# medvedevgroup/TwoPaCo

Measured on AMD Instinct MI355X. Metric: kmers_hashed_per_sec, higher is better.
Workload: dtype u64

## Files before the change

### twopaco_amd/csrc/tpc_capi.hip

```cpp
#include "tpc_ctx.h"

namespace tpch {

int fail(tpc_ctx *c, int code, const char *fmt, ...)
{
    char buf[512];
    va_list ap;
    va_start(ap, fmt);
    vsnprintf(buf, sizeof buf, fmt, ap);
    va_end(ap);
    if (c) c->err = buf;
    return code;
}





TpcLaunch make_launch(const tpc_ctx *c)
{
    TpcLaunch a;
    a.P = c->P; a.tab = c->tab; a.bases = c->bases; a.nmask = c->nmask; a.n_text = c->n_text;
    a.n_tiles = c->n_tiles; a.filter = c->filter; a.stream = c->stream;
    a.stat_kernel = c->stat_kernel;
    return a;
}

TpcLaunch make_launch_periodic(const tpc_ctx *c)
{
    TpcLaunch a = make_launch(c);
    if (c->periodic && c->periodic_valid) {
        if (c->periodic_any_q) a.per_qs = c->periodic;
        if (c->periodic_any_i) a.per_i = c->periodic + (size_t)(1 + TPC_PER_PLANES) * c->n_words_alloc;
    }
    return a;
}

void ensure_periodic(tpc_ctx *c)
{
    if (c->periodic_valid || !c->opt_periodic || !c->bases || !c->have_params || c->n_words_alloc == 0) return;
    if ((c->sh_world > 1 || c->text_windowed) && !c->opt_shard_periodic && !replicated(c)) return;
    TpcLaunch a = make_launch(c);
    const uint64_t w0 = c->text_windowed ? c->text_w0 : 0, w1 = c->text_windowed ? std::min(c->text_w1, c->n_words) : c->n_words;
    const uint64_t pos_hi = c->text_windowed ? c->text_w1 << 5 : ~0ull;
    uint32_t any[2] = {0, 0};
    uint32_t *flags = reinterpret_cast<uint32_t *>(c->counters + 6);
    if (hipMemsetAsync(flags, 0, sizeof any, c->stream) != hipSuccess) return;
    tpc_launch_periodic_build(a, nullptr, nullptr, 0, nullptr, w0, w1, w0 << 5, pos_hi, flags);
    if (hipMemcpyAsync(any, flags, sizeof any, hipMemcpyDeviceToHost, c->stream) != hipSuccess || hipStreamSynchronize(c->stream) != hipSuccess) return;
    c->periodic_any_q = any[0] != 0; c->periodic_any_i = any[1] != 0;
    if (any[0] || any[1]) {
        const size_t words = (size_t)(2 + TPC_PER_PLANES) * c->n_words_alloc;
        if (!c->periodic && hipMalloc((void **)&c->periodic, words * sizeof(uint32_t)) != hipSuccess) { (void)hipGetLastError(); c->periodic = nullptr; return; }
        if (hipMemsetAsync(c->periodic, 0, words * sizeof(uint32_t), c->stream) != hipSuccess) return;
        tpc_launch_periodic_build(a, c->periodic, c->periodic + c->n_words_alloc, c->n_words_alloc, c->periodic + (size_t)(1 + TPC_PER_PLANES) * c->n_words_alloc, w0, w1, w0 << 5, pos_hi, flags);
        if (hipStreamSynchronize(c->stream) != hipSuccess) return;
    }
// ... 194 lines not shown
        n = c->rmask_sums_n;
    } else {
        c->rmask_sums_valid = false;
        tpc_launch_mask_count(c->stream, m, c->n_words, c->block_sums, c->counters + 2);
        if ((rc = read_counter(c, 2, &n))) return rc;
    }
    rc = ensure(c, c->marks, c->marks_cap, n);
    if (rc) return rc;
    if (n) tpc_launch_mask_scatter(c->stream, m, c->n_words, c->block_sums, c->marks);
    c->n_marks = n;
    return 0;
}

}

extern "C" {

int tpc_ctx_create(int device, tpc_ctx **out)
{
    if (!out) return -1;
    *out = nullptr;
    int n = 0;
    if (hipGetDeviceCount(&n) != hipSuccess || n <= 0) return -2;
    if (device < 0 || device >= n) return -3;
    if (hipSetDevice(device) != hipSuccess) return -4;
    tpc_ctx *c = new tpc_ctx();
    c->device = device;
    c->dbg_ovf = getenv("TPC_DEBUG_OVF") != nullptr; c->dbg_phases = getenv("TPC_PROFILE_PHASES") != nullptr; c->dbg_timing = getenv("TWOPACO_TIMING") != nullptr; c->no_lean = TpcEnv::get().no_lean;
    if (const char *e = getenv("TPC_SHARD_TIGHT")) c->opt_shard_tight = atoi(e) ? 1 : 0;
    if (hipStreamCreate(&c->stream) != hipSuccess) { delete c; return -5; }
    for (int i = 0; i < TPC_K_COUNT; i++) {
        if (hipEventCreate(&c->ev0[i]) != hipSuccess || hipEventCreate(&c->ev1[i]) != hipSuccess) { delete c; return -5; }
    }
    if (hipMalloc((void **)&c->tab, TPC_TAB_WORDS * sizeof(uint64_t)) != hipSuccess ||
        hipMalloc((void **)&c->counters, 8 * sizeof(unsigned long long)) != hipSuccess ||
        hipMalloc((void **)&c->route_scratch, 128 * sizeof(unsigned long long)) != hipSuccess) { delete c; return -6; }
    *out = c;
    return 0;
}

void tpc_ctx_destroy(tpc_ctx *c)
{
    if (!c) return;
    (void)hipSetDevice(c->device);
    (void)hipStreamSynchronize(c->stream);
    void *ptrs[] = { c->tab, c->bases_alloc, c->nmask_alloc, c->filter, c->rmask, c->mask, c->marks, c->block_sums, c->table,
                     c->keys, c->idtab, c->emit_id, c->stream_buf, c->counters, c->route_scratch, c->sh_off, c->scan_blocks, c->sort_scratch, c->seg.name, c->seg.first, c->seg.ev[0], c->seg.ev[1], c->seg.ev[2],
                     c->seg.rec, c->seg.amb, c->text_plan.off, c->text_plan.piece, c->text_names, c->text_win };
    for (void *p : ptrs) if (p) (void)hipFree(p);
    stream_part_release(c);
    colors_drop(c);
    links_drop(c);
    anchors_drop(c);
    edges_drop(c);
    for (void *p : c->pbuf) if (p) (void)hipFree(p);
    for (void *p : c->ikeep) if (p) (void)hipFree(p);
    if (c->periodic) (void)hipFree(c->periodic);
    if (c->cmb_base) (void)hipFree(c->cmb_base);
    if (c->cmb_cur) (void)hipFree(c->cmb_cur);
    if (c->ikeep_ovf) (void)hipFree(c->ikeep_ovf);
    if (c->iovf_cnt) (void)hipFree(c->iovf_cnt);
    if (c->iovf_off) (void)hipFree(c->iovf_off);
    for (int i = 0; i < TPC_K_COUNT; i++) { if (c->ev0[i]) (void)hipEventDestroy(c->ev0[i]); if (c->ev1[i]) (void)hipEventDestroy(c->ev1[i]); }
    if (c->stream2) (void)hipStreamDestroy(c->stream2);
    if (c->stream) (void)hipStreamDestroy(c->stream);
    delete c;
}

const char *tpc_last_error(const tpc_ctx *c) { return c ? c->err.c_str() : "null context"; }

int tpc_set_option(tpc_ctx *c, const char *name, int64_t value)
{
    if (!c || !name) return -1;
    if (!strcmp(name, "insert_test_first")) { c->opt_test_first = value != 0; return 0; }
    if (!strcmp(name, "insert_mode")) { c->opt_insert_mode = (int)value; return 0; }
    if (!strcmp(name, "slice_bits")) { c->opt_slice_bits = (int)value; return 0; }
    if (!strcmp(name, "query_mode")) { c->opt_query_mode = (int)value; return 0; }
    if (!strcmp(name, "part_budget_bytes")) { c->opt_part_budget = value; return 0; }
    if (!strcmp(name, "part_levels")) { c->opt_part_levels = (int)value; return 0; }
    if (!strcmp(name, "shard_tight_regions")) { c->opt_shard_tight = value ? 1 : 0; c->sh_have[0] = c->sh_have[1] = false; return 0; }
    if (!strcmp(name, "part_min_tiles")) { c->opt_part_min_tiles = value < 1 ? 1 : value; return 0; }
    if (!strcmp(name, "verify_marks")) { c->opt_verify_marks = value != 0; return 0; }
    if (!strcmp(name, "mark_bucket_bits")) { tpc_test_mark_bucket_bits = (int)value; return 0; }
    if (!strcmp(name, "mark_region_cap")) { tpc_test_mark_region_cap = (int)value; return 0; }
    if (!strcmp(name, "mark_slice_bits")) { tpc_test_mark_slice_bits = (int)value; return 0; }
    if (!strcmp(name, "qhash_pushes")) { tpc_opt_qhash_pushes = value == 8 ? 8 : 6; return 0; }
    if (!strcmp(name, "qhash_roll_scalars")) { tpc_opt_qhash_roll = value != 0; return 0; }
    if (!strcmp(name, "fuse_apply_lookup")) { c->opt_fuse = value != 0; return 0; }
    if (!strcmp(name, "test_q6_pb2")) { tpc_test_q6_pb2 = (int)value; return 0; }
    if (!strcmp(name, "insert_entry_fmt")) { tpc_test_insert_p3 = value == 3; return 0; }
    if (!strcmp(name, "shard_periodic_skip")) { c->opt_shard_periodic = value != 0; return 0; }
    if (!strcmp(name, "periodic_skip")) { c->opt_periodic = value != 0; if (!value) c->periodic_valid = false; return 0; }
    if (!strcmp(name, "test_tight_pinch")) { tpc_test_tight_pinch = (int)value; c->sh_have[0] = c->sh_have[1] = false; return 0; }
    if (!strcmp(name, "test_sched_cap")) { tpc_test_sched_cap = value > 0 ? (uint32_t)value : 0; return 0; }
    if (!strcmp(name, "text_window")) { c->opt_text_window = value != 0; return 0; }
    if (!strcmp(name, "replicate_filter")) { c->opt_replicate = value != 0; return 0; }
    if (!strcmp(name, "test_force_anyq")) { tpc_test_force_anyq = value != 0; return 0; }
    if (!strcmp(name, "test_sketch_grid")) { tpc_test_sketch_grid = value > 0 ? (int)value : 0; return 0; }
    if (!strcmp(name, "test_links_slots_log2")) { c->opt_links_slots_log2 = (int)std::max<int64_t>(-1, std::min<int64_t>(value, 64)); return 0; }
    if (!strcmp(name, "test_edges_slots_log2")) { c->opt_edges_slots_log2 = (int)std::max<int64_t>(-1, std::min<int64_t>(value, 64)); return 0; }
    if (!strcmp(name, "test_edges_hash_bits")) { c->opt_edges_hash_bits = (int)std::max<int64_t>(-1, std::min<int64_t>(value, 65)); return 0; }
    if (!strcmp(name, "test_locate_grid")) { c->opt_locate_grid = value > 0 ? (int)std::min<int64_t>(value, 1 << 20) : 0; return 0; }
    if (!strcmp(name, "test_distances_chunk_words")) { c->opt_distances_chunk_words = (int)std::max<int64_t>(-1, std::min<int64_t>(value, 1 << 20)); return 0; }
    if (!strcmp(name, "test_components_step_limit")) { c->opt_components_step_limit = (int)std::max<int64_t>(-1, std::min<int64_t>(value, 0x7FFFFFFF)); return 0; }
    if (!strcmp(name, "test_fail_mallocs")) { tpc_test_fail_mallocs.store(value > 0 ? (int)value : 0); return 0; }
    return fail(c, -1, "unknown option %s", name);
}

int tpc_preload(int device)
{
    if (hipSetDevice(device) != hipSuccess) { (void)hipGetLastError(); return -10; }
    const bool timing = getenv("TWOPACO_TIMING") != nullptr;
    int (*const warm[4])() = { tpc_warm_partition, tpc_warm_qpartition, tpc_warm_pass2, tpc_warm_stream };
    const char *const name[4] = { "partition", "qpartition", "pass2", "stream" };
    for (int i = 0; i < 4; i++) {
        const auto t0 = std::chrono::steady_clock::now();
        if (warm[i]() != 0) return -10;
        if (timing) fprintf(stderr, "[timing]     code object %s: %.1f ms\n", name[i], std::chrono::duration<double, std::milli>(std::chrono::steady_clock::now() - t0).count());
    }
    return 0;
}

int tpc_warmup(tpc_ctx *c)
{
    if (!c) return -1;
    return tpc_preload(c->device);
}

int64_t tpc_get_stat(const tpc_ctx *c, const char *name)
{
    if (!c || !name) return -1;
    if (!strcmp(name, "insert_path")) return c->stat_path[0];
    if (!strcmp(name, "query_path")) return c->stat_path[1];
    if (!strcmp(name, "insert_entry_fmt")) return c->stat_fmt[0];
    if (!strcmp(name, "query_entry_fmt")) return c->stat_fmt[1];
    if (!strcmp(name, "insert_hash_kernel")) return c->stat_kernel[0];
    if (!strcmp(name, "query_hash_kernel")) return c->stat_kernel[1];
    if (!strcmp(name, "query_verify_kernel")) return c->stat_kernel[2];
    if (!strcmp(name, "query_hash_form")) return c->stat_kernel[3];
    if (!strcmp(name, "query_mark_path")) return c->stat_mark_path;
    if (!strcmp(name, "query_mark_fallback")) return c->stat_mark_fallback;
    if (!strcmp(name, "insert_batches")) return c->stat_batches[0];
    if (!strcmp(name, "query_batches")) return c->stat_batches[1];
    if (!strcmp(name, "query_tiles_per_batch")) return c->stat_q_plan[0];
    if (!strcmp(name, "query_b1")) return c->stat_q_plan[1];
    if (!strcmp(name, "query_b2")) return c->stat_q_plan[2];
    if (!strcmp(name, "query_begun")) return c->stat_q_begun;
    if (!strcmp(name, "filter2_retries")) return c->stat_filter2_retries;
    if (!strcmp(name, "aggregate_retries")) return c->stat_aggregate_retries;
    if (!strcmp(name, "filter2_counted")) return c->stat_filter2_counted;
    if (!strcmp(name, "fused_lookups")) return c->stat_fused;
    if (!strcmp(name, "query_overflow_entries")) return c->stat_query_overflow;
    if (!strcmp(name, "insert_overflow_entries")) return c->stat_insert_overflow;
    if (!strcmp(name, "periodic_skip")) return c->periodic_valid ? 1 : 0;
    if (!strcmp(name, "pbuf_releases")) return c->stat_pbuf_releases;
    if (!strcmp(name, "distances_tile")) return TPC_DISTANCES_TILE;
    if (!strcmp(name, "text_words")) return (int64_t)(c->text_w1 - c->text_w0);
    if (!strcmp(name, "text_word_begin")) return (int64_t)c->text_w0;
    if (!strcmp(name, "text_word_end")) return (int64_t)c->text_w1;
    if (!strcmp(name, "periodic_any_query")) return c->periodic_valid && c->periodic_any_q ? 1 : 0;
    if (!strcmp(name, "periodic_any_insert")) return c->periodic_valid && c->periodic_any_i ? 1 : 0;
    if (!strcmp(name, "text_write_us")) return c->text_write_us;
    if (!strcmp(name, "text_wait_us")) return c->text_wait_us;
    if (!strcmp(name, "text_window_bytes")) return c->text_window_bytes;
    if (!strcmp(name, "device_free_bytes") || !strcmp(name, "device_total_bytes")) {
        size_t free_b = 0, total_b = 0;
        if (hipSetDevice(c->device) != hipSuccess || hipMemGetInfo(&free_b, &total_b) != hipSuccess) { (void)hipGetLastError(); return -1; }
        return (int64_t)(name[7] == 'f' ? free_b : total_b);
    }
    if (!strcmp(name, "round_marks")) return c->marks_valid ? (int64_t)c->n_marks : -1;
    return -1;
}

int tpc_set_params(tpc_ctx *c, int k, int L, int q, const uint64_t *seed_table)
{
    if (!c || !seed_table) return -1;
    if (q < 1 || q > TPC_MAX_Q) return fail(c, -1, "q=%d unsupported (1..%d)", q, TPC_MAX_Q);
    if (L < 2 || L > 62) return fail(c, -1, "filter bits L=%d unsupported (2..62)", L);
    if (k < 1) return fail(c, -1, "k must be positive");
    const int C = (k + 4 + 31) / 32;
    if (C >= 20)
        return fail(c, -1, "The value of K is too big. Please refer to documentaion how to increase the max supported value of K.");
    HIPCHK(c, hipSetDevice(c->device));
    c->P.k = k; c->P.L = L; c->P.q = q; c->P.rk = k % L; c->P.lmask = (1ull << L) - 1ull;
    if (C != c->C && c->keys) {
        (void)hipFree(c->keys);
        c->keys = nullptr; c->keys_cap = 0;
    }
    c->C = C;
    memset(c->tab_host, 0, sizeof c->tab_host);
    for (int i = 0; i < q; i++)
        for (int ch = 0; ch < 5; ch++) {
            const uint64_t h = seed_table[i * 5 + ch];
            if (h > c->P.lmask) return fail(c, -1, "seed table entry exceeds L bits");
            c->tab_host[i * 5 + ch] = h;
            c->tab_host[TPC_TAB_HK + i * 5 + ch] = rotln_host(h, L, c->P.rk);
        }
    HIPCHK(c, hipMemcpy(c->tab, c->tab_host, sizeof c->tab_host, hipMemcpyHostToDevice));
    const uint64_t fw = filter_words_for(L, c->opt_replicate ? 1 : c->sh_world);
    c->sh_have[0] = c->sh_have[1] = false;
    c->pending_lists = false; c->cmb_have_geo = false;
    if (fw != c->filter_words) {
        if (c->filter) (void)hipFree(c->filter);
        c->filter = nullptr;
        HIPCHK(c, hipMalloc((void **)&c->filter, fw * sizeof(uint32_t)));
        c->filter_words = fw;
    }
    c->have_params = true;
    c->periodic_valid = false;
    c->pending_apply = false;
    c->qb_valid = false;
    c->n_keys = 0; c->finalized = false; c->rounds_done = 0; c->mask_dirty = false; c->marks_valid = false; c->rmask_sums_valid = false;
    return 0;
}

int tpc_seq_upload(tpc_ctx *c, const uint64_t *bases, const uint32_t *nmask, uint64_t n_text)
{
    if (!c || !bases || !nmask || n_text < 2) return fail(c, -1, "bad text");
    HIPCHK(c, hipSetDevice(c->device));
    const auto t_begin = std::chrono::steady_clock::now();
    c->qb_valid = false;
    const uint64_t nw = (n_text + 31) / 32;
    if (!((nmask[0] & 1u) && ((nmask[(n_text - 1) >> 5] >> ((n_text - 1) & 31)) & 1u)))
        return fail(c, -1, "text must start and end with the N separator");
    const uint64_t tiles = (nw + TPC_TILE_THREADS - 1) / TPC_TILE_THREADS;
    const uint64_t alloc = ((n_text / TPC_RUN + 512) / 512) * 512 + TPC_XW_MAX + 2;
    uint64_t w0 = 0, w1 = alloc;
    const bool windowed = c->opt_text_window && c->sh_world > 1;
    if (windowed) {
        const uint64_t t512 = (n_text / TPC_RUN + 512) / 512, chunk = (t512 + c->sh_world - 1) / c->sh_world;
// ... 609 lines not shown
```

### twopaco_amd/csrc/tpc_ctx.h

```cpp
#pragma once
#include "../../include/twopaco_hip.h"
#include "tpc_internal.h"

#include <algorithm>
#include <atomic>
#include <cmath>
#include <chrono>
#include <cstdarg>
#include <cstdio>
#include <cstdlib>
#include <cstring>
#include <string>
#include <vector>
#include <map>

struct tpc_ctx {
    __attribute__((always_inline)) tpc_ctx() = default;
    int device = 0;
    hipStream_t stream = nullptr;
    std::string err;
    bool have_params = false;
    TpcHashParams P{};
    uint64_t tab_host[TPC_TAB_WORDS]{};
    uint64_t *tab = nullptr;
    int C = 1;
    uint64_t *bases = nullptr;
    uint32_t *nmask = nullptr;
    uint64_t n_text = 0, n_words = 0, n_words_alloc = 0, n_tiles = 0;
    uint64_t text_uploads = 0;
    uint32_t *periodic = nullptr;
    bool periodic_valid = false;
    bool periodic_any_q = false, periodic_any_i = false;
    int opt_periodic = 1;
    bool opt_shard_periodic = false;
    uint64_t *bases_alloc = nullptr;
    uint32_t *nmask_alloc = nullptr;
    int opt_text_window = 0;
    bool text_windowed = false;
    uint64_t text_w0 = 0, text_w1 = 0;
    uint32_t *filter = nullptr;
    uint64_t filter_words = 0;
    uint32_t *rmask = nullptr, *mask = nullptr;
    bool mask_dirty = false;
    int rounds_done = 0;
    uint64_t *marks = nullptr;
    uint64_t marks_cap = 0, n_marks = 0;
    bool marks_valid = false;
    bool rmask_sums_valid = false;
    uint64_t rmask_sums_n = 0;
    uint64_t *block_sums = nullptr;
    uint64_t *scan_blocks = nullptr;
    void *table = nullptr;
    uint64_t table_cap = 0, table_alloc = 0;
    uint64_t *keys = nullptr;
    uint64_t n_keys = 0, keys_cap = 0;
    bool finalized = false;
// ... 97 lines not shown
        bool valid = false;
    } edg;
    struct Locate {
        unsigned long long *hit = nullptr;
        uint32_t *row = nullptr;
        uint32_t *runs = nullptr;
        unsigned long long *recs = nullptr;
        unsigned long long *shared = nullptr;
        uint64_t positions = 0, windows = 0, found = 0, n_runs = 0, n_rec = 0, peak_bytes = 0;
        uint32_t n_colors = 0;
        bool valid = false;
    } loc;
    int opt_edges_slots_log2 = 0;
    int opt_edges_hash_bits = 0;
    int opt_locate_grid = 0;
    int opt_components_step_limit = 0;
    int opt_distances_chunk_words = 0;
    unsigned long long *counters = nullptr;
    unsigned long long *route_scratch = nullptr;
    uint64_t *sh_off = nullptr;
    size_t sh_off_bytes = 0;
    int opt_test_first = 0;
    int opt_insert_mode = 0;
    int opt_slice_bits = 20;
    bool filter_zero_pending = false;
    static constexpr int NPBUF = 19;
    void *pbuf[NPBUF] = {};
    size_t pbytes[NPBUF] = {};
    std::vector<uint64_t> off2_uploaded, off3_uploaded;
    int opt_part_levels = 0;
    int opt_shard_tight = 1;
    int stat_path[2] = {0, 0};
    int64_t stat_batches[2] = {0, 0};
    mutable int stat_kernel[4] = {0, 0, 0, 0};
    int stat_fmt[2] = {0, 0};
    int64_t stat_filter2_retries = 0;
    int64_t stat_aggregate_retries = 0;
    int stat_filter2_counted = 0;
    int opt_verify_marks = 1;
    int stat_mark_path = 0;
    int64_t stat_mark_fallback = 0;
    int64_t opt_part_min_tiles = 256;
    int64_t opt_part_budget = 0;
    int opt_query_mode = 0;
    int opt_fuse = 1;
    bool pending_apply = false;
    bool pending_fresh = false;
    bool pending_shard = false;
    TpcPartPlan pending_pl;
    void *ikeep[2] = {nullptr, nullptr};
    size_t ikeep_bytes[2] = {0, 0};
    uint64_t *ikeep_ovf = nullptr;
    uint64_t ikeep_ovf_cap = 0;
    uint64_t pending_novf = 0;
    uint32_t *iovf_cnt = nullptr;
    uint64_t *iovf_off = nullptr;
    uint32_t iovf_slices = 0;
    int64_t stat_fused = 0;
    int64_t stat_query_overflow = 0;
    int64_t stat_insert_overflow = 0;
    int64_t stat_pbuf_releases = 0;
    uint32_t sh_rank = 0, sh_world = 1;
    TpcPartPlan sh_ipl;
    TpcQPlan sh_qpl;
    bool sh_have[2] = {false, false};
    uint64_t sh_per[2] = {0, 0}, sh_batches[2] = {0, 0};
    uint64_t sh_nsurv = 0;
// ... 91 lines not shown
```

### twopaco_amd/csrc/tpc_internal.h

```cpp
#pragma once
#include "tpc_device.h"
#include <algorithm>
#include <cstdlib>
#include <vector>

struct TpcEnv {
    bool no_lean, rb_hash, verify_eager, gated_full;
    int verify_marks;
    int qhash_pushes, qhash_roll;
    int ppr_insert, gated_loads, split_loads9;
    int slice_grid;
    static const TpcEnv &get()
    {
        static const TpcEnv e = [] {
            TpcEnv v;
            v.no_lean = getenv("TPC_NO_LEAN") != nullptr;
            v.rb_hash = getenv("TPC_RB_HASH") != nullptr;
            const char *lz = getenv("TPC_VERIFY_LAZY");
            v.verify_eager = lz && lz[0] == '0';
            v.gated_full = getenv("TPC_GATED_FULL_REGIONS") != nullptr;
            const char *vm = getenv("TPC_VERIFY_MARKS");
            v.verify_marks = vm && vm[0] ? (vm[0] != '0' ? 1 : 0) : -1;
            const char *qp = getenv("TPC_QHASH_PUSHES");
            v.qhash_pushes = qp && (atoi(qp) == 6 || atoi(qp) == 8) ? atoi(qp) : 0;
            const char *qr = getenv("TPC_QHASH_ROLL_SCALARS");
            v.qhash_roll = qr && qr[0] ? (qr[0] != '0' ? 1 : 0) : -1;
            const char *p = getenv("TPC_PPR_INSERT"), *g = getenv("TPC_GATED_LOADS");
            v.ppr_insert = p ? atoi(p) : 0;
            v.gated_loads = g ? atoi(g) : 0;
            const char *s9 = getenv("TPC_SPLIT_LOADS9");
            v.split_loads9 = s9 ? atoi(s9) : 0;
            const char *lg = getenv("TPC_LOOKUP_GRID");
            int n_cu = 0, dev = 0;
            if (hipGetDevice(&dev) != hipSuccess || hipDeviceGetAttribute(&n_cu, hipDeviceAttributeMultiprocessorCount, dev) != hipSuccess || n_cu <= 0) { (void)hipGetLastError(); n_cu = 256; }
            v.slice_grid = lg ? atoi(lg) : 2 * n_cu;
            return v;
        }();
        return e;
    }
};

inline uint32_t tpc_slice_grid(uint32_t n_slices)
{
    const int g = TpcEnv::get().slice_grid;
    return g > 0 ? std::min<uint32_t>(n_slices, (uint32_t)g) : n_slices;
}

extern int tpc_opt_qhash_pushes, tpc_opt_qhash_roll;
inline bool tpc_qhash_roll_scalars() { const int e = TpcEnv::get().qhash_roll; return (e >= 0 ? e : tpc_opt_qhash_roll) != 0; }
inline bool tpc_qhash_compact() { const int e = TpcEnv::get().qhash_pushes; return (e ? e : tpc_opt_qhash_pushes) != 8; }

#define TPC_TAB_MAXQ 64
#define TPC_KERNEL_MAXQ 16
#define TPC_TAB_HK (TPC_TAB_MAXQ * 5)
#define TPC_TAB_WORDS (2 * TPC_TAB_MAXQ * 5)

struct TpcLaunch {
    TpcHashParams P;
    const uint64_t *tab;
    const uint64_t *bases;
    const uint32_t *nmask;
    uint64_t n_text;
    uint64_t n_tiles;
    uint32_t *filter;
    hipStream_t stream;
    const uint32_t *per_i = nullptr, *per_qs = nullptr;
    uint64_t g_begin = 0, g_end = ~0ull;
    hipEvent_t ev_lookup0 = nullptr, ev_lookup1 = nullptr;
    int *stat_kernel = nullptr;
};
constexpr int TPC_PER_MAXP = 63;
constexpr int TPC_PER_PLANES = 6;
int tpc_launch_periodic_build(const TpcLaunch &a, uint32_t *qs, uint32_t *qd, uint64_t stride, uint32_t *ins, uint64_t w_begin, uint64_t w_end, uint64_t pos_lo, uint64_t pos_hi,
                              uint32_t *any);
int tpc_launch_periodic_copy(hipStream_t stream, uint32_t *rmask, const uint32_t *qs, const uint32_t *qd, uint64_t stride, uint64_t n_words);

int tpc_launch_insert(const TpcLaunch &a, uint64_t lo, uint64_t hi, bool gated, bool test, unsigned long long *n_kmers);
int tpc_launch_query(const TpcLaunch &a, uint32_t *rmask, uint64_t lo, uint64_t hi, bool gated, unsigned long long *n_marks);
int tpc_launch_split(const TpcLaunch &a, uint32_t *emask, uint32_t *bins, uint64_t bin_size);
int tpc_launch_split_emask(hipStream_t s, const uint64_t *d_rec_start, const uint64_t *d_rec_len, uint32_t n_rec, int k, uint64_t n_words, uint32_t *emask);
int tpc_launch_hash_dump(const TpcLaunch &a, uint64_t g0, uint64_t n, uint64_t *out);
int tpc_launch_insert_anyq(const TpcLaunch &a, uint64_t lo, uint64_t hi, bool gated, bool test, unsigned long long *n_kmers);
int tpc_launch_query_anyq(const TpcLaunch &a, uint32_t *rmask, uint64_t lo, uint64_t hi, bool gated, unsigned long long *n_marks);
int tpc_launch_split_anyq(const TpcLaunch &a, uint32_t *emask, uint32_t *bins, uint64_t bin_size);
extern int tpc_test_force_anyq;

struct TpcPartPlan {
    int slice_bits, b1, b2, pos_per_round;
    int b3 = 0;
    uint32_t perm_mult, perm_inv;
    uint64_t tile0, n_tiles;
    uint32_t nwg1, wpb;
// ... 207 lines not shown
```

### twopaco_amd/csrc/tpc_qpartition.hip

```cpp
#ifndef TPC_QPARTITION_PART
#define TPC_QPARTITION_PART 0
#endif
#include "tpc_rbins.h"
#include "tpc_bins3.h"
#include "tpc_binsp.h"
#include "tpc_lean.h"
#include "tpc_internal.h"
#include "tpc_lists.h"
#include <algorithm>
#include <type_traits>
#include <cstdio>
#include <cstdlib>
#include <cmath>

#if TPC_QPARTITION_PART == 0
int tpc_test_q6_pb2 = 0;
int tpc_opt_qhash_pushes = 6, tpc_opt_qhash_roll = 1;
int tpc_test_mark_bucket_bits = 0, tpc_test_mark_region_cap = 0, tpc_test_mark_slice_bits = 0;
#endif

namespace {

constexpr int QE_E_SHIFT = 31;
constexpr uint64_t QE_REM_MASK = (1ull << QE_E_SHIFT) - 1ull;
constexpr int QS_LISTS = 64;

struct QOverflow {
    uint64_t *list;
    unsigned long long *cursor;
    uint64_t cap;
    __device__ __forceinline__ void push(uint64_t addr, uint64_t sid, int site = 0) const
    {
#ifdef TPC_PROFILE_PHASES
        atomicAdd(cursor + 24 + site, 1ull);
#endif
        const unsigned long long o = atomicAdd(cursor, 1ull);
        if (o < cap) { list[2 * o] = addr; list[2 * o + 1] = sid; } else cursor[1] = 1ull;
    }
};

__device__ __forceinline__ bool within(uint64_t v, uint64_t lo, uint64_t hi) { return v >= lo && v <= hi; }

constexpr int QH_THREADS = 1024;
constexpr int QH_RUN = 16;

__device__ __forceinline__ uint64_t q_rotl_n(uint64_t x, int L, int r)
{
    if (r == 0) return x;
    return ((x & ((1ull << (L - r)) - 1ull)) << r) | (x >> (L - r));
}
// ... 110 lines not shown
#pragma unroll
                            for (int c = 0; c < 4; c++) {
                                {
                                    const uint64_t a0 = perm.fwd(tpc_min(hk0[c] ^ v.pos[0], r1n ^ h0[3 - c]));
                                    eb[c] = (uint32_t)(a0 >> shift);
                                    ev[c] = (a0 & (((uint64_t)1 << shift) - 1)) | ((sid_g | (uint64_t)c) << QE_E_SHIFT);
                                    eok[c] = c != c_prev;
                                }
                                {
                                    const uint64_t a0 = perm.fwd(tpc_min(r1p ^ h0[c], v.neg[0] ^ hk0[3 - c]));
                                    eb[4 + c] = (uint32_t)(a0 >> shift);
                                    ev[4 + c] = (a0 & (((uint64_t)1 << shift) - 1)) | ((sid_g | (uint64_t)(4 + c)) << QE_E_SHIFT);
                                    eok[4 + c] = c != c_next;
                                }
                            }
                            bins.template push_batch<8>(eb, ev, eok, lost);
                        }
                    }
                    v.pos[0] = r1p ^ s_h[c_next] ^ s_hk[c_first];
                    v.neg[0] = tpc_rotr1(v.neg[0] ^ s_hk[tpc_rc(c_next)] ^ s_h[tpc_rc(c_first)], P.L);
                    ncnt += (c_next == TPC_CODE_N) - (c_first == TPC_CODE_N);
                    c_prev = c_first;
                    c_first = c_first_nx;
                }
            }
            bins.template flush<false>(lost);
        }
        rmask16[(wfirst * 2) + tid] = (uint16_t)word;
    }
    if constexpr (RB) { bins.flush(true, reg, lost); bins.store_counts(cnt1, reg, ridx); }
    else { bins.template flush<true>(lost); bins.store_counts(cnt1, ridx); }
}

constexpr int QT_MAXK = 64;
constexpr uint32_t QH_ROLL_S = 1u;

__device__ __forceinline__ uint64_t q_spread2(uint32_t m)
{
    uint64_t x = m;
    x = (x | (x << 16)) & 0x0000FFFF0000FFFFull;
    x = (x | (x << 8)) & 0x00FF00FF00FF00FFull;
    x = (x | (x << 4)) & 0x0F0F0F0F0F0F0F0Full;
    x = (x | (x << 2)) & 0x3333333333333333ull;
    x = (x | (x << 1)) & 0x5555555555555555ull;
    return x | (x << 1);
}

template <bool GATED, bool SHARDED, bool HALF, bool LHI, bool PUSH6>
__global__ void __launch_bounds__(QH_THREADS)
k_q_hash2(int LOG_NB, TpcHashParams P, const uint64_t *__restrict__ tab, const uint64_t *__restrict__ bases,
          const uint32_t *__restrict__ nmask, uint64_t n_text, uint64_t tile0, uint64_t n_tiles, int pos_per_round,
          uint64_t lo, uint64_t hi, uint64_t *buf1, uint32_t *cnt1, uint64_t cap1, QOverflow ovf, PtPerm perm, PtShard sh,
          uint64_t gbase, uint32_t *__restrict__ rmask, uint32_t tiles_per_wg, const uint16_t *__restrict__ skip16, uint32_t mode)
{
    using V = LeanV<LHI>;
    extern __shared__ __attribute__((aligned(16))) unsigned char smem[];
    const int NB = 1 << LOG_NB;
    constexpr int TW = PT_THREADS + 1 + TPC_XW_MAX;
    Bins3<uint64_t, QH_THREADS> bins;
    uint64_t *s_b = reinterpret_cast<uint64_t *>(bins.carve(smem, LOG_NB));
    uint64_t *s_roll = s_b + TW;
    uint64_t *s_seed = s_roll + 20;
    uint32_t *s_n = reinterpret_cast<uint32_t *>(s_seed + QT_MAXK * 10);
    const uint32_t tid = threadIdx.x;
    const int k = P.k, L = P.L;
    if (tid < 5) {
        const uint32_t c = tid, rc = c == 4 ? 4u : 3u - c;
        s_roll[c * 2] = tab[c]; s_roll[c * 2 + 1] = tab[TPC_TAB_HK + rc];
        s_roll[10 + c * 2] = tab[TPC_TAB_HK + c]; s_roll[10 + c * 2 + 1] = tab[rc];
    }
    if (k <= QT_MAXK)
        for (uint32_t i = tid; i < 5u * (uint32_t)k; i += QH_THREADS) {
            const uint32_t t = i / 5u, c = i % 5u, rc = c == 4 ? 4u : 3u - c;
            s_seed[2 * i] = q_rotl_n(tab[c], L, (k - 1 - (int)t) % L);
            s_seed[2 * i + 1] = q_rotl_n(tab[rc], L, (int)t % L);
        }
    const int shift = L - LOG_NB;
    const uint32_t wg = blockIdx.x, nwg = gridDim.x;
    auto ridx = [sh, NB, wg, nwg](uint32_t b) { return SHARDED ? pt_r1_send(sh, (uint32_t)NB, nwg, wg, b) : (uint64_t)wg * NB + b; };
    auto lost = [shift, ovf](uint32_t b, uint64_t val) { ovf.push(((uint64_t)b << shift) | (val & QE_REM_MASK), val >> QE_E_SHIFT, 1); };
    bins.init(buf1, [cap1, ridx](uint32_t b) { return make_uint2((uint32_t)((ridx(b) * cap1) >> 4), (uint32_t)cap1); });
    LeanRotH<LHI> R;
    R.set(L);
    LeanSplit S;
    S.set(perm, LOG_NB);
    const int xw = (k + 1) / 32 + 2;
    uint16_t *rmask16 = reinterpret_cast<uint16_t *>(rmask);
    uint32_t h0l[5], h0h[5], hk0l[5], hk0h[5];
#pragma unroll
    for (int c = 0; c < 5; c++) {
        const uint64_t h = tab[c], hk = tab[TPC_TAB_HK + c];
        h0l[c] = (uint32_t)h; h0h[c] = (uint32_t)(h >> 32); hk0l[c] = (uint32_t)hk; hk0h[c] = (uint32_t)(hk >> 32);
    }
    auto pick = [](uint32_t c, const uint32_t (&x)[5], const uint32_t (&y)[5], uint32_t &ox, uint32_t &oy) {
        const bool b0 = (c & 1u) != 0u, b1 = (c & 2u) != 0u, n = c >= 4u;
        const uint32_t x01 = b0 ? x[1] : x[0], x23 = b0 ? x[3] : x[2], y32 = b0 ? y[2] : y[3], y10 = b0 ? y[0] : y[1];
        const uint32_t xv = b1 ? x23 : x01, yv = b1 ? y10 : y32;
        ox = n ? x[4] : xv; oy = n ? y[4] : yv;
    };
    const uint32_t ppr_mask = (uint32_t)pos_per_round - 1u;
    constexpr bool half_rounds = HALF;
    const uint32_t p0 = 32u + tid * (uint32_t)QH_RUN;
    const uint64_t t_first = tile0 + (tiles_per_wg ? (uint64_t)blockIdx.x * tiles_per_wg : (uint64_t)blockIdx.x);
    const uint64_t t_end = tiles_per_wg ? min(tile0 + n_tiles, t_first + tiles_per_wg) : tile0 + n_tiles;
    const uint64_t t_step = tiles_per_wg ? 1u : gridDim.x;
    for (uint64_t tile = t_first; tile < t_end; tile += t_step) {
        const uint64_t wfirst = tile * PT_THREADS;
        __syncthreads();
        const uint32_t sk = skip16 ? (uint32_t)skip16[(wfirst * 2) + tid] : 0u;
        for (int i = (int)tid; i < PT_THREADS + 1 + xw; i += QH_THREADS) {
            const int64_t w = (int64_t)wfirst - 1 + i;
            uint64_t b = w >= 0 ? bases[w] : 0ull;
            const uint32_t m = w >= 0 ? nmask[w] : 0xFFFFFFFFu;
            if (m) b &= ~q_spread2(m);
            s_b[i] = b;
            s_n[i] = m;
        }
        __syncthreads();
        const uint32_t cw = lean_chars16(s_b, p0), nw = lean_nbits32(s_n, p0);
        const uint32_t cx = lean_chars16(s_b, p0 + (uint32_t)k), nx = lean_nbits32(s_n, p0 + (uint32_t)k);
        uint32_t cp = lean_char(s_b, s_n, p0 - 1u);
        int ncnt = 0;
        for (int t = 0; t < k; t += 32) {
            uint32_t bits = lean_nbits32(s_n, p0 + (uint32_t)t);
            if (k - t < 32) bits &= (1u << (k - t)) - 1u;
            ncnt += __popc(bits);
        }
        V pos = lv_make<LHI>(0u, 0u), neg = lv_make<LHI>(0u, 0u);
        if (k <= QT_MAXK) {
            for (int t0 = 0; t0 < k; t0 += 16) {
                uint32_t ch = lean_chars16(s_b, p0 + (uint32_t)t0), nb = lean_nbits32(s_n, p0 + (uint32_t)t0);
                const int m = min(16, k - t0);
                const uint4 *row = reinterpret_cast<const uint4 *>(s_seed) + t0 * 5;
                for (int j = 0; j < m; j++) {
                    const uint32_t c = (ch & 3u) | ((nb & 1u) << 2);
                    ch >>= 2; nb >>= 1;
                    const uint4 e = row[j * 5 + c];
                    pos = lv_xor<LHI>(pos, e.x, e.y);
                    neg = lv_xor<LHI>(neg, e.z, e.w);
                }
            }
        } else {
            for (int t = 0; t < k; t++) {
                const uint32_t c = lean_char(s_b, s_n, p0 + (uint32_t)t), cr = lean_char(s_b, s_n, p0 + (uint32_t)(k - 1 - t));
                pos = lv_xor<LHI>(R.rotl1(pos), lv_from64<LHI>(s_roll[c * 2]));
                neg = lv_xor<LHI>(R.rotl1(neg), lv_from64<LHI>(s_roll[10 + cr * 2 + 1]));
            }
        }
        const uint32_t sid0 = ((uint32_t)(wfirst * TPC_RUN + (uint64_t)tid * QH_RUN - gbase) | (SHARDED ? sh.rank << (30u - sh.log_world()) : 0u)) << 2;
        uint32_t word = 0;
#pragma unroll 1
        for (int s = 0; s < QH_RUN; s++) {
            const uint32_t cf = __builtin_amdgcn_ubfe(cw, 2u * (uint32_t)s, 2u) | (__builtin_amdgcn_ubfe(nw, (uint32_t)s, 1u) << 2);
            const uint32_t cn = __builtin_amdgcn_ubfe(cx, 2u * (uint32_t)s, 2u) | (__builtin_amdgcn_ubfe(nx, (uint32_t)s, 1u) << 2);
            const V r1p = R.rotl1(pos), r1n = R.rotl1(neg);
            bool check = ncnt == 0;
            if (GATED) check = check && within(lv_u64<LHI>(lv_min<LHI>(pos, neg)), lo, hi);
            const bool nadj = (cp | cn) >= 4u;
            if (check && nadj) word |= 1u << s;
            uint32_t eb[8];
            uint64_t ev[8];
            bool eok[8];
// ... 27 lines not shown
                        const uint32_t b3[3] = {b6[0], b6[1], b6[2]};
                        const uint64_t v3[3] = {v6[0], v6[1], v6[2]};
                        bins.template push_batch<3>(b3, v3, all3, lost);
                    }
                } else if constexpr (!half_rounds) bins.template push_batch<8>(eb, ev, eok, lost);
                else {
                    uint32_t b4[4];
                    uint64_t v4[4];
                    bool o4[4];
#pragma unroll
                    for (int c = 0; c < 4; c++) { b4[c] = eb[c]; v4[c] = ev[c]; o4[c] = eok[c]; }
                    bins.template push_batch<4>(b4, v4, o4, lost);
                }
                probing = true;
            }
            if constexpr (half_rounds) {
                bins.template flush<false>(lost);
                if (probing) {
                    if constexpr (PUSH6) {
                        const uint32_t b3[3] = {b6[3], b6[4], b6[5]};
                        const uint64_t v3[3] = {v6[3], v6[4], v6[5]};
                        bins.template push_batch<3>(b3, v3, all3, lost);
                    } else {
                        uint32_t b4[4];
                        uint64_t v4[4];
                        bool o4[4];
#pragma unroll
                        for (int c = 0; c < 4; c++) { b4[c] = eb[4 + c]; v4[c] = ev[4 + c]; o4[c] = eok[4 + c]; }
                        bins.template push_batch<4>(b4, v4, o4, lost);
                    }
                }
            }
            if (s + 1 < QH_RUN) {
                uint4 en, ef;
                if ((PUSH6 || !SHARDED) && (mode & QH_ROLL_S)) {
                    pick(cn, h0l, hk0l, en.x, en.z); pick(cf, hk0l, h0l, ef.x, ef.z);
                    en.y = en.w = ef.y = ef.w = 0u;
                    if constexpr (LHI) { pick(cn, h0h, hk0h, en.y, en.w); pick(cf, hk0h, h0h, ef.y, ef.w); }
                } else {
                    en = reinterpret_cast<const uint4 *>(s_roll)[cn]; ef = reinterpret_cast<const uint4 *>(s_roll)[5 + cf];
                }
                pos = lv_xor<LHI>(lv_xor<LHI>(r1p, en.x, en.y), ef.x, ef.y);
                neg = R.rotr1(lv_xor<LHI>(lv_xor<LHI>(neg, en.z, en.w), ef.z, ef.w));
                ncnt += (int)(cn >> 2) - (int)(cf >> 2);
                cp = cf;
            }
            if ((((uint32_t)s + 1u) & ppr_mask) == 0u) bins.template flush<false>(lost);
        }
        rmask16[(wfirst * 2) + tid] = (uint16_t)word;
    }
    bins.template flush<true>(lost);
    bins.store_counts(cnt1, ridx);
}

constexpr int QS_THREADS = 1024;
template <bool SHARDED, bool RB, bool P6 = false>
__global__ void __launch_bounds__(QS_THREADS)
k_q_split(int LOG_NB1, int LOG_NB2, int L, int slice_bits, int loads, uint32_t nwg1, uint32_t wpb, const uint64_t *__restrict__ buf1,
          const uint32_t *__restrict__ cnt1, uint64_t cap1, uint64_t *buf2, uint32_t *cnt2, const uint64_t *__restrict__ off2, QOverflow ovf,
          PtShard sh, uint32_t prev_wpb, int log_prev_nb2, uint32_t nreg_cap, uint32_t sched_cap, const uint64_t *__restrict__ off1,
          const uint64_t *__restrict__ own1, const uint32_t *__restrict__ owncnt1, uint32_t *__restrict__ bnd = nullptr, uint32_t n_groups = 0,
          uint32_t tiles_per_wg = 0, uint32_t batch_tiles = 0, uint32_t pb2 = 0)
{
    extern __shared__ __attribute__((aligned(16))) unsigned char smem[];
    const uint32_t NB1 = 1u << LOG_NB1, NB2 = 1u << LOG_NB2;
    constexpr int LOADS = P6 ? 5 : 4;
    constexpr uint64_t SENT = ~0ull;
    static_assert(!P6 || (!SHARDED && !RB), "the 6-byte output is the one-rank, flush-per-round form");
    typename std::conditional<P6, BinsP<PFmt6, QS_THREADS>,
                              typename std::conditional<RB, RBins<uint64_t, QS_THREADS>, Bins3<uint64_t, QS_THREADS>>::type>::type bins;
    uint64_t *s_off = reinterpret_cast<uint64_t *>(bins.carve(smem, LOG_NB2));
    if constexpr (RB) bins.init();
    else {
        const uint64_t *o2 = off2 + (uint64_t)blockIdx.x * NB2;
        if constexpr (P6) bins.init(buf2, [o2](uint32_t b) { const uint64_t o = o2[b]; return make_uint2((uint32_t)o, (uint32_t)(o2[b + 1] - o)); });
        else bins.init(buf2, [o2](uint32_t b) { const uint64_t o = o2[b]; return make_uint2((uint32_t)(o >> 4), (uint32_t)(o2[b + 1] - o)); });
// ... 915 lines not shown
            if (own[u] >= 0) {
                const uint64_t slot = base[own[u]] + rank[u];
                dst[slot] = val[u] & keep;
                if (perm) perm[i] = (uint32_t)slot;
            }
        }
        __syncthreads();
    }
}

__global__ void __launch_bounds__(256)
k_route_count64(const uint64_t *__restrict__ v, uint64_t n, int shift, uint32_t omask, unsigned long long *counts)
{
    __shared__ uint32_t h[RT_MAXW];
    if (threadIdx.x < RT_MAXW) h[threadIdx.x] = 0;
    __syncthreads();
    const uint64_t stride = (uint64_t)gridDim.x * blockDim.x;
    for (uint64_t i = (uint64_t)blockIdx.x * blockDim.x + threadIdx.x; i < n; i += stride) atomicAdd(&h[(uint32_t)(v[i] >> shift) & omask & (RT_MAXW - 1)], 1u);
    __syncthreads();
    if (threadIdx.x < RT_MAXW && h[threadIdx.x]) atomicAdd(&counts[threadIdx.x], (unsigned long long)h[threadIdx.x]);
}

#endif
#if TPC_QPARTITION_PART == 0
inline bool q_use_rbins(int log_nb) { return log_nb >= 9; }

void launch_qhash(const TpcLaunch &a, const TpcQPlan &pl, bool gated, uint64_t lo, uint64_t hi, uint32_t *rmask)
{
    QOverflow ovf{pl.ovf, pl.ovf_cur, pl.ovf_cap};
    const PtPerm perm{pl.slice_bits, pl.b1 + pl.b2 + pl.b3, pl.perm_mult, pl.perm_inv};
    const PtShard sh{pl.rank, pl.world};
    const bool rb = q_use_rbins(pl.b1);
    const bool lean = pl.b1 <= 9 && pl.sub_rounds <= 2 && perm.F <= 24 && !TpcEnv::get().no_lean && !(rb && TpcEnv::get().rb_hash);
    if (a.stat_kernel) { a.stat_kernel[1] = lean ? 1 : 2; a.stat_kernel[3] = 0; }
    if (lean) {
        const size_t lds = Bins3<uint64_t, QH_THREADS>::lds_bytes(pl.b1) + (size_t)(PT_THREADS + 1 + TPC_XW_MAX) * 12 + 160 + (size_t)QT_MAXK * 80 + 64;
        const uint32_t mode = tpc_qhash_roll_scalars() && (tpc_qhash_compact() || pl.world == 1) ? QH_ROLL_S : 0u;
        if (a.stat_kernel) a.stat_kernel[3] = (tpc_qhash_compact() ? 1 : 0) | (mode & QH_ROLL_S ? 2 : 0) | (gated ? 4 : 0);
#define TPC_QHASH2_GO(G, S, H, X, C)                                                                                                          \
    do {                                                                                                                                    \
        (void)hipFuncSetAttribute((const void *)k_q_hash2<G, S, H, X, C>, hipFuncAttributeMaxDynamicSharedMemorySize, (int)lds);               \
        hipLaunchKernelGGL((k_q_hash2<G, S, H, X, C>), dim3(pl.nwg1), dim3(QH_THREADS), lds, a.stream, pl.b1, a.P, a.tab, a.bases, a.nmask, a.n_text, \
                           pl.tile0, pl.n_tiles, pl.pos_per_round, lo, hi, pl.buf1, pl.cnt1, pl.cap1, ovf, perm, sh,                          \
                           pl.tile0_global * (uint64_t)(PT_THREADS * TPC_RUN), rmask, pl.fmt == 6 ? pl.tiles_per_wg : 0u,                  \
                           reinterpret_cast<const uint16_t *>(a.per_qs),            \
                           mode);                                                                                                          \
    } while (0)
#define TPC_QHASH2_GS(H, X, C)                                                                                                              \
    do {                                                                                                                                    \
        if (pl.world > 1) { if (gated) TPC_QHASH2_GO(true, true, H, X, C); else TPC_QHASH2_GO(false, true, H, X, C); }                      \
        else { if (gated) TPC_QHASH2_GO(true, false, H, X, C); else TPC_QHASH2_GO(false, false, H, X, C); }                                 \
    } while (0)
#define TPC_QHASH2_HX(C)                                                                                                                    \
    do {                                                                                                                                    \
        if (a.P.L > 32) { if (pl.b1 >= 9) TPC_QHASH2_GS(true, true, C); else TPC_QHASH2_GS(false, true, C); }                               \
        else { if (pl.b1 >= 9) TPC_QHASH2_GS(true, false, C); else TPC_QHASH2_GS(false, false, C); }                                        \
    } while (0)
        if (tpc_qhash_compact()) TPC_QHASH2_HX(true); else TPC_QHASH2_HX(false);
#undef TPC_QHASH2_HX
#undef TPC_QHASH2_GS
#undef TPC_QHASH2_GO
        return;
    }
    const size_t lds = (rb ? RBins<uint64_t, QH_THREADS>::lds_bytes(pl.b1) : Bins3<uint64_t, QH_THREADS>::lds_bytes(pl.b1)) +
                       (size_t)(PT_THREADS + 1 + TPC_XW_MAX) * 12 + (size_t)5 * 16 + 64;
#define TPC_QHASH_GO(G, S, R)                                                                                                               \
    do {                                                                                                                                    \
        (void)hipFuncSetAttribute((const void *)k_q_hash<G, S, R>, hipFuncAttributeMaxDynamicSharedMemorySize, (int)lds);                   \
        hipLaunchKernelGGL((k_q_hash<G, S, R>), dim3(pl.nwg1), dim3(QH_THREADS), lds, a.stream, pl.b1, a.P, a.tab, a.bases, a.nmask, a.n_text,  \
                           pl.tile0, pl.n_tiles, pl.pos_per_round, pl.sub_rounds, lo, hi, pl.buf1, pl.cnt1, pl.cap1, ovf, perm, sh,              \
                           pl.tile0_global * (uint64_t)(PT_THREADS * TPC_RUN), rmask);                                                      \
    } while (0)
#define TPC_QHASH_GS(R)                                                                                                                     \
    do {                                                                                                                                    \
        if (pl.world > 1) { if (gated) TPC_QHASH_GO(true, true, R); else TPC_QHASH_GO(false, true, R); }                                    \
        else { if (gated) TPC_QHASH_GO(true, false, R); else TPC_QHASH_GO(false, false, R); }                                               \
    } while (0)
    if (rb) TPC_QHASH_GS(true); else TPC_QHASH_GS(false);
#undef TPC_QHASH_GS
// ... 831 lines not shown
```

Measured before the change: 12.51 billion.

## Precompute per-position seed hash table on host and use branchless masked XOR in query hash

```diff
diff --git a/twopaco_amd/csrc/tpc_capi.hip b/twopaco_amd/csrc/tpc_capi.hip
--- a/twopaco_amd/csrc/tpc_capi.hip
+++ b/twopaco_amd/csrc/tpc_capi.hip
@@ -23,6 +23,7 @@
     a.P = c->P; a.tab = c->tab; a.bases = c->bases; a.nmask = c->nmask; a.n_text = c->n_text;
     a.n_tiles = c->n_tiles; a.filter = c->filter; a.stream = c->stream;
     a.stat_kernel = c->stat_kernel;
+    if (c->P.k <= TPC_QSEED_MAXK) a.qseed = c->tab + TPC_TAB_WORDS;
     return a;
 }
 
@@ -283,7 +284,7 @@
     for (int i = 0; i < TPC_K_COUNT; i++) {
         if (hipEventCreate(&c->ev0[i]) != hipSuccess || hipEventCreate(&c->ev1[i]) != hipSuccess) { delete c; return -5; }
     }
-    if (hipMalloc((void **)&c->tab, TPC_TAB_WORDS * sizeof(uint64_t)) != hipSuccess ||
+    if (hipMalloc((void **)&c->tab, sizeof c->tab_host) != hipSuccess ||
         hipMalloc((void **)&c->counters, 8 * sizeof(unsigned long long)) != hipSuccess ||
         hipMalloc((void **)&c->route_scratch, 128 * sizeof(unsigned long long)) != hipSuccess) { delete c; return -6; }
     *out = c;
@@ -337,6 +338,7 @@
     if (!strcmp(name, "mark_slice_bits")) { tpc_test_mark_slice_bits = (int)value; return 0; }
     if (!strcmp(name, "qhash_pushes")) { tpc_opt_qhash_pushes = value == 8 ? 8 : 6; return 0; }
     if (!strcmp(name, "qhash_roll_scalars")) { tpc_opt_qhash_roll = value != 0; return 0; }
+    if (!strcmp(name, "qhash_seed_scalars")) { tpc_opt_qhash_seed = value != 0; return 0; }
     if (!strcmp(name, "fuse_apply_lookup")) { c->opt_fuse = value != 0; return 0; }
     if (!strcmp(name, "test_q6_pb2")) { tpc_test_q6_pb2 = (int)value; return 0; }
     if (!strcmp(name, "insert_entry_fmt")) { tpc_test_insert_p3 = value == 3; return 0; }
@@ -389,6 +391,8 @@
     if (!strcmp(name, "query_hash_kernel")) return c->stat_kernel[1];
     if (!strcmp(name, "query_verify_kernel")) return c->stat_kernel[2];
     if (!strcmp(name, "query_hash_form")) return c->stat_kernel[3];
+    if (!strcmp(name, "query_hash_seed")) return c->stat_kernel[4];
+    if (!strcmp(name, "query_hash_seed_maxk")) return TPC_QSEED_MAXK;
     if (!strcmp(name, "query_mark_path")) return c->stat_mark_path;
     if (!strcmp(name, "query_mark_fallback")) return c->stat_mark_fallback;
     if (!strcmp(name, "insert_batches")) return c->stat_batches[0];
@@ -447,6 +451,13 @@
             c->tab_host[i * 5 + ch] = h;
             c->tab_host[TPC_TAB_HK + i * 5 + ch] = rotln_host(h, L, c->P.rk);
         }
+    if (k <= TPC_QSEED_MAXK)
+        for (int t = 0; t < k; t++)
+            for (int ch = 0; ch < 5; ch++) {
+                const int rc = ch == 4 ? 4 : 3 - ch;
+                c->tab_host[TPC_TAB_WORDS + (t * 5 + ch) * 2] = rotln_host(c->tab_host[ch], L, (k - 1 - t) % L);
+                c->tab_host[TPC_TAB_WORDS + (t * 5 + ch) * 2 + 1] = rotln_host(c->tab_host[rc], L, t % L);
+            }
     HIPCHK(c, hipMemcpy(c->tab, c->tab_host, sizeof c->tab_host, hipMemcpyHostToDevice));
     const uint64_t fw = filter_words_for(L, c->opt_replicate ? 1 : c->sh_world);
     c->sh_have[0] = c->sh_have[1] = false;
diff --git a/twopaco_amd/csrc/tpc_ctx.h b/twopaco_amd/csrc/tpc_ctx.h
--- a/twopaco_amd/csrc/tpc_ctx.h
+++ b/twopaco_amd/csrc/tpc_ctx.h
@@ -21,7 +21,7 @@
     std::string err;
     bool have_params = false;
     TpcHashParams P{};
-    uint64_t tab_host[TPC_TAB_WORDS]{};
+    uint64_t tab_host[TPC_TAB_WORDS + TPC_QSEED_WORDS]{};
     uint64_t *tab = nullptr;
     int C = 1;
     uint64_t *bases = nullptr;
@@ -185,7 +185,7 @@
     int opt_shard_tight = 1;
     int stat_path[2] = {0, 0};
     int64_t stat_batches[2] = {0, 0};
-    mutable int stat_kernel[4] = {0, 0, 0, 0};
+    mutable int stat_kernel[5] = {0, 0, 0, 0, 0};
     int stat_fmt[2] = {0, 0};
     int64_t stat_filter2_retries = 0;
     int64_t stat_aggregate_retries = 0;
diff --git a/twopaco_amd/csrc/tpc_internal.h b/twopaco_amd/csrc/tpc_internal.h
--- a/twopaco_amd/csrc/tpc_internal.h
+++ b/twopaco_amd/csrc/tpc_internal.h
@@ -7,7 +7,7 @@
 struct TpcEnv {
     bool no_lean, rb_hash, verify_eager, gated_full;
     int verify_marks;
-    int qhash_pushes, qhash_roll;
+    int qhash_pushes, qhash_roll, qhash_seed;
     int ppr_insert, gated_loads, split_loads9;
     int slice_grid;
     static const TpcEnv &get()
@@ -25,6 +25,8 @@
             v.qhash_pushes = qp && (atoi(qp) == 6 || atoi(qp) == 8) ? atoi(qp) : 0;
             const char *qr = getenv("TPC_QHASH_ROLL_SCALARS");
             v.qhash_roll = qr && qr[0] ? (qr[0] != '0' ? 1 : 0) : -1;
+            const char *qs = getenv("TPC_QHASH_SEED_SCALARS");
+            v.qhash_seed = qs && qs[0] ? (qs[0] != '0' ? 1 : 0) : -1;
             const char *p = getenv("TPC_PPR_INSERT"), *g = getenv("TPC_GATED_LOADS");
             v.ppr_insert = p ? atoi(p) : 0;
             v.gated_loads = g ? atoi(g) : 0;
@@ -46,18 +48,22 @@
     return g > 0 ? std::min<uint32_t>(n_slices, (uint32_t)g) : n_slices;
 }
 
-extern int tpc_opt_qhash_pushes, tpc_opt_qhash_roll;
+extern int tpc_opt_qhash_pushes, tpc_opt_qhash_roll, tpc_opt_qhash_seed;
 inline bool tpc_qhash_roll_scalars() { const int e = TpcEnv::get().qhash_roll; return (e >= 0 ? e : tpc_opt_qhash_roll) != 0; }
+inline bool tpc_qhash_seed_scalars() { const int e = TpcEnv::get().qhash_seed; return (e >= 0 ? e : tpc_opt_qhash_seed) != 0; }
 inline bool tpc_qhash_compact() { const int e = TpcEnv::get().qhash_pushes; return (e ? e : tpc_opt_qhash_pushes) != 8; }
 
 #define TPC_TAB_MAXQ 64
 #define TPC_KERNEL_MAXQ 16
 #define TPC_TAB_HK (TPC_TAB_MAXQ * 5)
 #define TPC_TAB_WORDS (2 * TPC_TAB_MAXQ * 5)
+#define TPC_QSEED_MAXK 64
+#define TPC_QSEED_WORDS (TPC_QSEED_MAXK * 5 * 2)
 
 struct TpcLaunch {
     TpcHashParams P;
     const uint64_t *tab;
+    const uint64_t *qseed = nullptr;
     const uint64_t *bases;
     const uint32_t *nmask;
     uint64_t n_text;
diff --git a/twopaco_amd/csrc/tpc_qpartition.hip b/twopaco_amd/csrc/tpc_qpartition.hip
--- a/twopaco_amd/csrc/tpc_qpartition.hip
+++ b/twopaco_amd/csrc/tpc_qpartition.hip
@@ -15,7 +15,7 @@
 
 #if TPC_QPARTITION_PART == 0
 int tpc_test_q6_pb2 = 0;
-int tpc_opt_qhash_pushes = 6, tpc_opt_qhash_roll = 1;
+int tpc_opt_qhash_pushes = 6, tpc_opt_qhash_roll = 1, tpc_opt_qhash_seed = 1;
 int tpc_test_mark_bucket_bits = 0, tpc_test_mark_region_cap = 0, tpc_test_mark_slice_bits = 0;
 #endif
 
@@ -192,8 +192,18 @@
     else { bins.template flush<true>(lost); bins.store_counts(cnt1, ridx); }
 }
 
-constexpr int QT_MAXK = 64;
+constexpr int QT_MAXK = TPC_QSEED_MAXK;
 constexpr uint32_t QH_ROLL_S = 1u;
+constexpr uint32_t QH_SEED_S = 2u;
+
+__device__ __forceinline__ uint32_t q_xor_and(uint32_t v, uint32_t row, uint32_t mask)
+{
+#if __has_builtin(__builtin_amdgcn_bitop3_b32)
+    return __builtin_amdgcn_bitop3_b32(row, mask, v, 0x6Au);
+#else
+    return v ^ (row & mask);
+#endif
+}
 
 __device__ __forceinline__ uint64_t q_spread2(uint32_t m)
 {
@@ -211,7 +221,8 @@
 k_q_hash2(int LOG_NB, TpcHashParams P, const uint64_t *__restrict__ tab, const uint64_t *__restrict__ bases,
           const uint32_t *__restrict__ nmask, uint64_t n_text, uint64_t tile0, uint64_t n_tiles, int pos_per_round,
           uint64_t lo, uint64_t hi, uint64_t *buf1, uint32_t *cnt1, uint64_t cap1, QOverflow ovf, PtPerm perm, PtShard sh,
-          uint64_t gbase, uint32_t *__restrict__ rmask, uint32_t tiles_per_wg, const uint16_t *__restrict__ skip16, uint32_t mode)
+          uint64_t gbase, uint32_t *__restrict__ rmask, uint32_t tiles_per_wg, const uint16_t *__restrict__ skip16, uint32_t mode,
+          const uint4 *__restrict__ qseed)
 {
     using V = LeanV<LHI>;
     extern __shared__ __attribute__((aligned(16))) unsigned char smem[];
@@ -229,7 +240,7 @@
         s_roll[c * 2] = tab[c]; s_roll[c * 2 + 1] = tab[TPC_TAB_HK + rc];
         s_roll[10 + c * 2] = tab[TPC_TAB_HK + c]; s_roll[10 + c * 2 + 1] = tab[rc];
     }
-    if (k <= QT_MAXK)
+    if (k <= QT_MAXK && !(mode & QH_SEED_S))
         for (uint32_t i = tid; i < 5u * (uint32_t)k; i += QH_THREADS) {
             const uint32_t t = i / 5u, c = i % 5u, rc = c == 4 ? 4u : 3u - c;
             s_seed[2 * i] = q_rotl_n(tab[c], L, (k - 1 - (int)t) % L);
@@ -252,11 +263,10 @@
         const uint64_t h = tab[c], hk = tab[TPC_TAB_HK + c];
         h0l[c] = (uint32_t)h; h0h[c] = (uint32_t)(h >> 32); hk0l[c] = (uint32_t)hk; hk0h[c] = (uint32_t)(hk >> 32);
     }
-    auto pick = [](uint32_t c, const uint32_t (&x)[5], const uint32_t (&y)[5], uint32_t &ox, uint32_t &oy) {
-        const bool b0 = (c & 1u) != 0u, b1 = (c & 2u) != 0u, n = c >= 4u;
-        const uint32_t x01 = b0 ? x[1] : x[0], x23 = b0 ? x[3] : x[2], y32 = b0 ? y[2] : y[3], y10 = b0 ? y[0] : y[1];
-        const uint32_t xv = b1 ? x23 : x01, yv = b1 ? y10 : y32;
-        ox = n ? x[4] : xv; oy = n ? y[4] : yv;
+    auto hot = [](uint32_t chars, uint32_t nbits, uint32_t i, uint32_t (&m)[5]) {
+        const uint32_t m0 = (uint32_t)__builtin_amdgcn_sbfe((int)chars, 2u * i, 1u), m1 = (uint32_t)__builtin_amdgcn_sbfe((int)chars, 2u * i + 1u, 1u);
+        m[4] = (uint32_t)__builtin_amdgcn_sbfe((int)nbits, i, 1u);
+        m[0] = ~(m0 | m1 | m[4]); m[1] = m0 & ~m1; m[2] = m1 & ~m0; m[3] = m0 & m1;
     };
     const uint32_t ppr_mask = (uint32_t)pos_per_round - 1u;
     constexpr bool half_rounds = HALF;
@@ -287,7 +297,27 @@
             ncnt += __popc(bits);
         }
         V pos = lv_make<LHI>(0u, 0u), neg = lv_make<LHI>(0u, 0u);
-        if (k <= QT_MAXK) {
+        if (mode & QH_SEED_S) {
+            for (int t0 = 0; t0 < k; t0 += 16) {
+                const uint32_t ch = lean_chars16(s_b, p0 + (uint32_t)t0), nb = lean_nbits32(s_n, p0 + (uint32_t)t0);
+                const int m = min(16, k - t0);
+                const uint4 *row = qseed + t0 * 5;
+                for (int j = 0; j < m; j++) {
+                    uint32_t mk[5];
+                    hot(ch, nb, (uint32_t)j, mk);
+                    const uint4 r0 = row[j * 5], r1 = row[j * 5 + 1], r2 = row[j * 5 + 2], r3 = row[j * 5 + 3], r4 = row[j * 5 + 4];
+                    auto mix = [&mk](uint32_t v, uint32_t a, uint32_t c, uint32_t g, uint32_t t, uint32_t x) {
+                        return q_xor_and(q_xor_and(q_xor_and(q_xor_and(q_xor_and(v, a, mk[0]), c, mk[1]), g, mk[2]), t, mk[3]), x, mk[4]);
+                    };
+                    pos.lo = mix(pos.lo, r0.x, r1.x, r2.x, r3.x, r4.x);
+                    neg.lo = mix(neg.lo, r0.z, r1.z, r2.z, r3.z, r4.z);
+                    if constexpr (LHI) {
+                        pos.hi = mix(pos.hi, r0.y, r1.y, r2.y, r3.y, r4.y);
+                        neg.hi = mix(neg.hi, r0.w, r1.w, r2.w, r3.w, r4.w);
+                    }
+                }
+            }
+        } else if (k <= QT_MAXK) {
             for (int t0 = 0; t0 < k; t0 += 16) {
                 uint32_t ch = lean_chars16(s_b, p0 + (uint32_t)t0), nb = lean_nbits32(s_n, p0 + (uint32_t)t0);
                 const int m = min(16, k - t0);
@@ -381,16 +411,26 @@
                 }
             }
             if (s + 1 < QH_RUN) {
-                uint4 en, ef;
                 if ((PUSH6 || !SHARDED) && (mode & QH_ROLL_S)) {
-                    pick(cn, h0l, hk0l, en.x, en.z); pick(cf, hk0l, h0l, ef.x, ef.z);
-                    en.y = en.w = ef.y = ef.w = 0u;
-                    if constexpr (LHI) { pick(cn, h0h, hk0h, en.y, en.w); pick(cf, hk0h, h0h, ef.y, ef.w); }
+                    uint32_t mnx[5], mfx[5];
+                    hot(cx, nx, (uint32_t)s, mnx); hot(cw, nw, (uint32_t)s, mfx);
+                    V p = r1p, q = neg;
+#pragma unroll
+                    for (int c = 0; c < 5; c++) {
+                        const int r = c == 4 ? 4 : 3 - c;
+                        p.lo = q_xor_and(q_xor_and(p.lo, h0l[c], mnx[c]), hk0l[c], mfx[c]);
+                        q.lo = q_xor_and(q_xor_and(q.lo, hk0l[r], mnx[c]), h0l[r], mfx[c]);
+                        if constexpr (LHI) {
+                            p.hi = q_xor_and(q_xor_and(p.hi, h0h[c], mnx[c]), hk0h[c], mfx[c]);
+                            q.hi = q_xor_and(q_xor_and(q.hi, hk0h[r], mnx[c]), h0h[r], mfx[c]);
+                        }
+                    }
+                    pos = p; neg = R.rotr1(q);
                 } else {
-                    en = reinterpret_cast<const uint4 *>(s_roll)[cn]; ef = reinterpret_cast<const uint4 *>(s_roll)[5 + cf];
+                    const uint4 en = reinterpret_cast<const uint4 *>(s_roll)[cn], ef = reinterpret_cast<const uint4 *>(s_roll)[5 + cf];
+                    pos = lv_xor<LHI>(lv_xor<LHI>(r1p, en.x, en.y), ef.x, ef.y);
+                    neg = R.rotr1(lv_xor<LHI>(lv_xor<LHI>(neg, en.z, en.w), ef.z, ef.w));
                 }
-                pos = lv_xor<LHI>(lv_xor<LHI>(r1p, en.x, en.y), ef.x, ef.y);
-                neg = R.rotr1(lv_xor<LHI>(lv_xor<LHI>(neg, en.z, en.w), ef.z, ef.w));
                 ncnt += (int)(cn >> 2) - (int)(cf >> 2);
                 cp = cf;
             }
@@ -1372,11 +1412,15 @@
     const PtShard sh{pl.rank, pl.world};
     const bool rb = q_use_rbins(pl.b1);
     const bool lean = pl.b1 <= 9 && pl.sub_rounds <= 2 && perm.F <= 24 && !TpcEnv::get().no_lean && !(rb && TpcEnv::get().rb_hash);
-    if (a.stat_kernel) { a.stat_kernel[1] = lean ? 1 : 2; a.stat_kernel[3] = 0; }
+    if (a.stat_kernel) { a.stat_kernel[1] = lean ? 1 : 2; a.stat_kernel[3] = 0; a.stat_kernel[4] = 0; }
     if (lean) {
         const size_t lds = Bins3<uint64_t, QH_THREADS>::lds_bytes(pl.b1) + (size_t)(PT_THREADS + 1 + TPC_XW_MAX) * 12 + 160 + (size_t)QT_MAXK * 80 + 64;
-        const uint32_t mode = tpc_qhash_roll_scalars() && (tpc_qhash_compact() || pl.world == 1) ? QH_ROLL_S : 0u;
-        if (a.stat_kernel) a.stat_kernel[3] = (tpc_qhash_compact() ? 1 : 0) | (mode & QH_ROLL_S ? 2 : 0) | (gated ? 4 : 0);
+        const uint32_t mode = (tpc_qhash_roll_scalars() && (tpc_qhash_compact() || pl.world == 1) ? QH_ROLL_S : 0u) |
+                              (tpc_qhash_seed_scalars() && a.qseed && a.P.k <= QT_MAXK ? QH_SEED_S : 0u);
+        if (a.stat_kernel) {
+            a.stat_kernel[3] = (tpc_qhash_compact() ? 1 : 0) | (mode & QH_ROLL_S ? 2 : 0) | (gated ? 4 : 0);
+            a.stat_kernel[4] = mode & QH_SEED_S ? 1 : 0;
+        }
 #define TPC_QHASH2_GO(G, S, H, X, C)                                                                                                          \
     do {                                                                                                                                    \
         (void)hipFuncSetAttribute((const void *)k_q_hash2<G, S, H, X, C>, hipFuncAttributeMaxDynamicSharedMemorySize, (int)lds);               \
@@ -1384,7 +1428,7 @@
                            pl.tile0, pl.n_tiles, pl.pos_per_round, lo, hi, pl.buf1, pl.cnt1, pl.cap1, ovf, perm, sh,                          \
                            pl.tile0_global * (uint64_t)(PT_THREADS * TPC_RUN), rmask, pl.fmt == 6 ? pl.tiles_per_wg : 0u,                  \
                            reinterpret_cast<const uint16_t *>(a.per_qs),            \
-                           mode);                                                                                                          \
+                           mode, reinterpret_cast<const uint4 *>(a.qseed));                                                                \
     } while (0)
 #define TPC_QHASH2_GS(H, X, C)                                                                                                              \
     do {                                                                                                                                    \
```

After: 12.78 billion (median of 6 runs). 1.02x the previous value.
